# duckdb/duckdb-vss

Measured on AMD Instinct MI355X. Metric: queries/sec at recall@10, 10M×768 FLOAT top-10; index build rows/sec, higher is better.
Workload: dtype f32

## Files before the change

duckdb-vss_amd/__init__.py:

```python
import ctypes as C
import os
import subprocess

import numpy as np

HERE = os.path.dirname(os.path.abspath(__file__))
ROOT = os.path.dirname(HERE)
LIB_PATH = os.environ.get("VSS_LIBRARY") or os.path.join(HERE, "libvssgpu.so")
CSRC = os.path.join(HERE, "csrc")

METRICS = {"l2sq": 0, "cosine": 1, "ip": 2}
FUNCTIONS = {"array_distance": 0, "array_cosine_distance": 1, "array_negative_inner_product": 2}
FREE_KEY = np.iinfo(np.int64).max

HIPCC_FLAGS = ["--offload-arch=gfx950", "-O3", "-std=c++17", "-ffp-contract=off", "-fPIC", "-Wno-int-to-pointer-cast"]


TRANSLATION_UNITS = ["vss_engine.hip", "vss_exchange.hip", "kernels_l2sq.hip", "kernels_cosine.hip", "kernels_ip.hip",
                     "kernels_boxes_l2sq.hip", "kernels_boxes_cosine.hip", "kernels_boxes_ip.hip",
                     "kernels_setboxes_l2sq.hip", "kernels_setboxes_cosine.hip", "kernels_setboxes_ip.hip"]


def build_library(force=False, extra_flags=(), out=None):
    out = out or os.path.join(HERE, "libvssgpu.so")
# ... 80 lines not shown
    "vss_set_label_column64": (_int, [_vp, _u32, _u64, _vp, _u64]),
    "vss_set_label_column64_device": (_int, [_vp, _u32, _u64, _vp, _u64]),
    "vss_label_column_width": (_u32, [_vp, _u32]),
    "vss_search_batch_by_label_box64": (_int, [_vp, _vp, _u64, _u64, _u64, _vp, _u64, _vp, _vp, _int, _u64, _vp, _vp, _vp, _vp]),
    "vss_search_batch_by_label_box64_device": (_int, [_vp, _vp, _u64, _u64, _u64, _vp, _u64, _vp, _vp, _int, _u64, _vp, _vp, _vp,
                                                      _vp]),
    "vss_search_batch_by_label_set_box": (_int, [_vp, _vp, _u64, _u64, _u64, _u32, _vp, _u32, _vp, _u64, _vp, _vp, _int, _u64, _vp, _vp,
                                                 _vp, _vp]),
    "vss_search_batch_by_label_set_box_device": (_int, [_vp, _vp, _u64, _u64, _u64, _u32, _vp, _u32, _vp, _u64, _vp, _vp, _int, _u64,
                                                        _vp, _vp, _vp, _vp]),
    "vss_last_exact_fallbacks": (_u64, [_vp]),
    "vss_last_search_stats": (_int, [_vp, _vp]),
    "vss_last_search_shape": (_int, [_vp, _vp]),
    "vss_last_search_prescore": (_int, [_vp, _vp]),
    "vss_last_search_prescore_descent": (_int, [_vp, _vp]),
    "vss_last_search_query_stats": (_int, [_vp, _vp, _u64]),
    "vss_timing": (_int, [_vp, _vp, _int]),
    "vss_build_work": (_int, [_vp, _vp]),
    "vss_remove_batch": (_int, [_vp, _vp, _u64, _vp]),
    "vss_compact": (_int, [_vp]),
    "vss_compact_ex": (_int, [_vp, _int, _vp]),
    "vss_size": (_u64, [_vp]),
    "vss_nodes": (_u64, [_vp]),
    "vss_build_progress": (_int, [_vp, _vp, _vp]),
    "vss_capacity": (_u64, [_vp]),
    "vss_max_level": (_u64, [_vp]),
    "vss_memory_usage": (_u64, [_vp]),
    "vss_dimensions": (_u64, [_vp]),
    "vss_metric": (_int, [_vp]),
    "vss_level_stats": (_int, [_vp, _u64, _vp]),
# ... 538 lines not shown

    def last_exact_fallbacks(self):
        return int(self.lib.vss_last_exact_fallbacks(self.h))

    def timing(self, reset=False):
        out = np.zeros(6, dtype=np.float64)
        self._check(self.lib.vss_timing(self.h, _p(out), int(reset)))
        return dict(search_kernel_ms=out[0], build_phase_a_ms=out[1], build_phase_b_ms=out[2], build_wall_ms=out[3],
                    build_batches=int(out[4]), build_retries=int(out[5]))

    def build_work(self):
        out = np.zeros(3, dtype=np.uint64)
        self._check(self.lib.vss_build_work(self.h, _p(out)))
        return dict(insert_distances=int(out[0]), insert_expansions=int(out[1]), link_distances=int(out[2]))

    def last_query_stats(self, nq):
        out = np.zeros((nq, 2), dtype=np.uint32)
        self._check(self.lib.vss_last_search_query_stats(self.h, _p(out), nq))
        return out

    def remove(self, rowids):
        rowids = np.ascontiguousarray(rowids, dtype=np.int64)
        n = _u64(0)
        self._check(self.lib.vss_remove_batch(self.h, _p(rowids), len(rowids), C.byref(n)))
        return n.value

    def compact(self, reorder=True):
        done = C.c_int(0)
        self._check(self.lib.vss_compact_ex(self.h, 1 if reorder else 0, C.byref(done)))
        return bool(done.value)
# ... 79 lines not shown
```

duckdb-vss_amd/csrc/hnsw_kernels.h:

```cpp
#pragma once
#include "wave_primitives.h"
#include "engine_layout.h"
#include "prescore_bound.h"
#include "filter_groups.h"
#include "label_filter.h"
#include <type_traits>

namespace vss {

constexpr int64_t FREE_KEY = 0x7FFFFFFFFFFFFFFFll;

constexpr uint64_t FILTER_PER_QUERY = 1ull << 63;
constexpr uint64_t FILTER_BY_LABEL = 1ull << 62;
constexpr uint64_t FILTER_BY_RANGE = 1ull << 61;
constexpr uint64_t FILTER_BY_SET = 1ull << 60;
constexpr uint64_t FILTER_FLAGS = FILTER_PER_QUERY | FILTER_BY_LABEL | FILTER_BY_RANGE | FILTER_BY_SET;
constexpr uint64_t FILTER_BY_BOX = FILTER_BY_RANGE | FILTER_BY_SET;
__host__ __device__ constexpr bool filter_by_box(uint64_t filter_bits) {
	return (filter_bits & FILTER_BY_BOX) == FILTER_BY_BOX;
}
constexpr uint64_t FILTER_BY_BOX64 = FILTER_BY_LABEL | FILTER_BY_RANGE | FILTER_BY_SET;
__host__ __device__ constexpr bool filter_by_box64(uint64_t filter_bits) {
	return (filter_bits & FILTER_BY_BOX64) == FILTER_BY_BOX64;
}
// ... 349 lines not shown
		return fresh;
	}
	__device__ __forceinline__ void clear_fresh() {
		fresh = 0;
	}
};

template <int MT, int NCH, int R, bool LATE = false>
struct SoloScorer {
	static constexpr bool touches_rows = LATE, touches_lists = LATE, helpers_touch = false;
	static constexpr bool bounds_descent = false;
	__device__ __forceinline__ void at_level(int) const {
	}
	__device__ __forceinline__ void at_bound(float) const {
	}
	__device__ __forceinline__ bool latency_mode() const {
		return false;
	}
	template <typename F>
	__device__ __forceinline__ void operator()(const WaveLds &lds, const RowSpace &sp, float qa2, int n, F before_loads
	                                           VSS_WC_ARG) const {
		if constexpr (LATE) {
			if (n <= 0)
				before_loads();
			wave_distances<MT, NCH, R>(sp, lds.q, qa2, lds.ids, n, lds.dist, before_loads);
		} else {
			before_loads();
			wave_distances<MT, NCH, R>(sp, lds.q, qa2, lds.ids, n, lds.dist);
		}
	}
// ... 4 lines not shown
	const int per = ((n + T - 1) / T + RG - 1) & ~(RG - 1);
	lo = wave * per < n ? wave * per : n;
	hi = lo + per < n ? lo + per : n;
}
struct NoListCache {};
template <int MT, int NCH, int R, int T>
struct TeamScorer {
	static constexpr bool touches_rows = false, touches_lists = true, helpers_touch = true;
	__device__ __forceinline__ bool latency_mode() const {
		return false;
	}
	static constexpr bool bounds_descent = false;
	__device__ __forceinline__ void at_level(int) const {
	}
	__device__ __forceinline__ void at_bound(float) const {
	}
	TeamBox *box;
	template <typename F, class Cache>
	__device__ __forceinline__ void run(const WaveLds &lds, const RowSpace &sp, float qa2, int n, F before_loads, Cache &cache,
	                                    bool touch) const {
		if (n <= 0) {
			before_loads();
			return;
		}
		if (lane_id() == 0)
			box->n = n, box->qa2 = qa2;
		__syncthreads();
		int lo, hi;
		team_share(sp, n, T, 0, lo, hi);
		wave_distances<MT, NCH, R>(sp, lds.q, qa2, lds.ids, hi, lds.dist, before_loads);
// ... 192 lines not shown
#pragma unroll
		for (int r = 0; r < RR; ++r)
			accumulate4<MT>(q, x[ch][r], ab[r], b2[r]);
	}
	transposed_reduce64<RR>(ab);
	if (MT == 1)
		transposed_reduce64<RR>(b2);
	constexpr int PER = 64 / RR;
	int j = pos[0];
#pragma unroll
	for (int r = 1; r < RR; ++r)
		j = (int)(lane / PER) == r ? pos[r] : j;
	if ((lane % PER) == 0)
		out[j] = finish_distance<MT>(ab[0], qa2, b2[0]);
}


typedef __attribute__((address_space(3))) unsigned long long lds_u64;
typedef __attribute__((address_space(3))) uint32_t lds_u32;
typedef __attribute__((address_space(3))) float lds_f32;
typedef uint32_t lds_u32x4 __attribute__((ext_vector_type(4)));
typedef __attribute__((address_space(3))) lds_u32x4 lds_u32x4_as3;
#define VSS_LDS_PTR(type, ptr) ((type *)(uint32_t)(uintptr_t)(ptr))
#define VSS_LDS_LOAD(type, ptr) __hip_atomic_load(VSS_LDS_PTR(type, ptr), __ATOMIC_RELAXED, __HIP_MEMORY_SCOPE_WORKGROUP)
#define VSS_LDS_STORE(type, ptr, v) __hip_atomic_store(VSS_LDS_PTR(type, ptr), (v), __ATOMIC_RELAXED, __HIP_MEMORY_SCOPE_WORKGROUP)
#define VSS_LDS_ADD(type, ptr, v) __hip_atomic_fetch_add(VSS_LDS_PTR(type, ptr), (v), __ATOMIC_RELAXED, __HIP_MEMORY_SCOPE_WORKGROUP)
#ifdef VSS_RELAXED_MAILBOX
#define VSS_MB_RELEASE __ATOMIC_RELAXED
#define VSS_MB_ACQUIRE __ATOMIC_RELAXED
#else
// ... 108 lines not shown
	uint32_t no_requests;
	uint32_t touch_ok;
	uint32_t prescore_ok;
	unsigned long long *descent_counters;
	mutable uint32_t crew_on = 0;
	mutable uint32_t level = 0;
	mutable float hop_bound = __builtin_inff();
	mutable uint32_t hop_filtered = 0;
	static constexpr bool bounds_descent = PRE;
	__device__ __forceinline__ void at_level(int l) const {
		level = (uint32_t)l;
	}
	__device__ __forceinline__ void at_bound(float bound) const {
		hop_bound = (PRE && descent_counters) ? bound : __builtin_inff();
	}
	__device__ __forceinline__ void add_descent_counts(uint32_t rows, uint32_t rejected) const {
		if (PRE && descent_counters && rows && lane_id() == 0) {
			atomicAdd(descent_counters, (unsigned long long)rows);
			atomicAdd(descent_counters + 1, (unsigned long long)rejected);
		}
	}

	__device__ __forceinline__ bool wants_requests() const {
		return !(crew_on && no_requests);
	}

	__device__ __forceinline__ bool latency_mode() const {
		return crew_on != 0 && touch_ok != 0;
	}
	__device__ __forceinline__ uint32_t active_walkers() const {
// ... 320 lines not shown
		VSS_TICK(tk1);
		VSS_ACC(t_pick, tk0, tk1);
		uint32_t first_cells;
		const bool have_first = can_prefetch && ahead.find(cs, first_cells);
		VSS_COUNT(t_look, have_first ? 1u : 0u);
		const int n = gather_neighbors<true>(gv, lds, cs, level, have_first, first_cells);
		VSS_TICK(tk2);
		VSS_ACC(t_gather, tk1, tk2);
		if (n < 0)
			return LEVEL_VISITED_OVERFLOW;
		auto look_ahead = request_ahead;
		if (n == 0) {
			look_ahead();
			continue;
		}
		if constexpr (TOUCH_H)
			score.run(lds, gv.sp, qa2, n, look_ahead, ahead, (lds.touch_lines & 0xFFu) && can_prefetch);
		else
			score(lds, gv.sp, qa2, n, look_ahead VSS_WC_PASS);
		wc.distances += n;
		VSS_TICK(tk3);
		VSS_ACC(t_dist, tk2, tk3);
		if constexpr (TOUCH) {
			if ((lds.touch_lines & 0xFFu) && can_prefetch) {
				touch.retire();
				VSS_COUNT(t_slice, (unsigned)__builtin_popcount(ahead.fresh_bits()));
				touch.issue(ahead, gv.sp, lds.touch_lines & 0xFFu);
			}
		}
		bool touch_lists = false;
// ... 317 lines not shown
				pool.end(nb, gv.sp, n_next);
			return LEVEL_INTERNAL;
		}
		if (next == EMPTY_SLOT)
			break;
		L.mark_expanded(pos);
		request_ahead();
		VSS_TICK(ta1);
		VSS_ACC(t_accept, ta0, ta1);
		b = nb;
		n_cur = n_next;
	}
	return LEVEL_OK;
}

template <int MT, int NCH, int R>
__device__ __forceinline__ int refine_candidates(const GraphView &gv, WaveLds &lds, int count, int needed,
                                                 WorkCounters &wc) {
	const int lane = lane_id();
	if (count < needed) {
		for (int i = lane; i < count; i += 64) {
			lds.kept_s[i] = lds.cand_s[i];
			lds.kept_d[i] = lds.cand_d[i];
		}
		wave_sync();
		return count;
	}
	if (lane == 0) {
		lds.kept_s[0] = lds.cand_s[0];
		lds.kept_d[0] = lds.cand_d[0];
	}
	wave_sync();
	int submitted = 1, consumed = 1;
	while (submitted < needed && consumed < count) {
		const uint32_t cs = lds.cand_s[consumed];
		const float cd = lds.cand_d[consumed];
		stage_row(lds.q2, gv.sp.vectors + (size_t)cs * gv.sp.V, gv.sp.V);
		const float c2 = MT == 1 ? wave_query_norm(gv.sp, lds.q2) : 0.f;
		const int pass = R * (64 >> gv.sp.logG);
		bool bad = false;
		for (int off = 0; off < submitted && !bad; off += pass) {
			const int n = submitted - off < pass ? submitted - off : pass;
			wave_distances<MT, NCH, R>(gv.sp, lds.q2, c2, lds.kept_s + off, n, lds.dist);
			wc.distances += n;
			for (int o = 0; o < n; o += 64) {
				const bool b = (o + lane < n) && (lds.dist[o + lane] < cd);
				bad = bad || (__ballot(b) != 0ull);
			}
			wave_sync();
		}
		if (!bad) {
			if (lane == 0) {
				lds.kept_s[submitted] = cs;
				lds.kept_d[submitted] = cd;
			}
			submitted++;
// ... 672 lines not shown
	uint32_t *counters;
	uint32_t req_capacity;
	uint32_t *global_hash;
	const uint32_t *work;
	uint32_t *node_status;
	uint32_t node_req_cap;
	unsigned long long *work_stats;
	const uint32_t *row_slot;
	const uint32_t *row_src;
	const float4 *pending;
	uint32_t *parked;
	uint32_t parked_stride;
	float *list_buf;
	uint32_t list_cap;
	uint32_t cand_lds_cap;
};

#ifndef VSS_BUILD_WAVES_PER_EU
#define VSS_BUILD_WAVES_PER_EU(NCH, E) ((NCH) == 6 ? 2 : (((E) >= 8 || (NCH) == 4) ? 3 : 4))
#endif
template <int MT, int NCH, int R, int E>
__global__ __launch_bounds__(64) __attribute__((amdgpu_waves_per_eu(VSS_BUILD_WAVES_PER_EU(NCH, E), 8))) void
k_build_phase_a(BuildArgs a) {
	extern __shared__ __attribute__((aligned(16))) unsigned char smem[];
	const int lane = lane_id();
	const uint32_t node = a.work ? a.work[blockIdx.x] : blockIdx.x;
	const uint32_t slot = a.row_slot ? a.row_slot[node] : a.first_slot + node;
	const uint32_t src = a.row_src ? a.row_src[node] : EMPTY_SLOT;
	WaveLds lds;
	carve_lds(lds, smem, a.hash_log2, a.gv.sp.V, a.list_cap_max, a.cand_lds_cap, a.global_hash);
	uint32_t *req_l = reinterpret_cast<uint32_t *>(
	    smem + wave_lds_bytes(a.hash_log2, a.gv.sp.V, a.list_cap_max, a.cand_lds_cap, a.global_hash == nullptr));
	float *req_dd = reinterpret_cast<float *>(req_l + a.node_req_cap);
	stage_row(lds.q, src == EMPTY_SLOT ? a.gv.sp.vectors + (size_t)slot * a.gv.sp.V : a.pending + (size_t)src * a.gv.sp.V,
	          a.gv.sp.V);
	const float qa2 = MT == 1 ? wave_query_norm(a.gv.sp, lds.q) : 0.f;
	WorkCounters wc = {};
	const int target = a.levels[slot];
	const SoloScorer<MT, NCH, R> score;
	uint32_t closest = descend<MT>(a.gv, lds, qa2, a.entry, a.max_level, target, score, wc);
	typename std::conditional<E == 0, MemList, WaveList<(E == 0 ? 1 : E)>>::type L;
	if constexpr (E == 0)
		L.bind(a.list_buf + (size_t)blockIdx.x * 2 * a.list_cap,
		       reinterpret_cast<uint32_t *>(a.list_buf + (size_t)blockIdx.x * 2 * a.list_cap) + a.list_cap);
	CandQueue unused_queue;
	uint32_t n_req = 0;
	for (int level = target < a.max_level ? target : a.max_level; level >= 0; --level) {
		if (level_search_impl<MT, true, false, 1>(a.gv, lds, qa2, closest, slot, level, a.top_limit, L, unused_queue, score, wc) !=
		    LEVEL_OK) {
			if (lane == 0) {
				a.node_status[node] = 1;
				atomicExch(&a.counters[3], 1u);
			}
			return;
		}
		if constexpr (E == 0) {
			for (int i = lane; i < L.size; i += 64)
				L.s[i] &= ~EXPANDED_BIT;
			lds.cand_d = L.d;
			lds.cand_s = L.s;
		} else {
			L.dump(lds.cand_d, lds.cand_s);
		}
		wave_sync();
		const int kept = refine_candidates<MT, NCH, R>(a.gv, lds, L.size, a.gv.M, wc);
		uint32_t *mine = src == EMPTY_SLOT ? a.gv.list_ptr(slot, level)
		                                   : a.parked + (size_t)node * a.parked_stride + (size_t)level * a.list_cap_max;
		const uint32_t cap = a.gv.list_cap(level);
		for (uint32_t i = lane; i < cap; i += 64)
			mine[i] = i < (uint32_t)kept ? lds.kept_s[i] : EMPTY_SLOT;
		for (int i = lane; i < kept; i += 64) {
			const uint32_t t = lds.kept_s[i];
			req_l[n_req + i] =
			    t == slot ? EMPTY_SLOT : (level == 0 ? t : a.gv.list_id_base + a.gv.upper_off[t] + (level - 1));
			req_dd[n_req + i] = lds.kept_d[i];
		}
		n_req += kept;
		closest = lds.kept_s[0];
		wave_sync();
	}
	uint32_t base = 0;
	if (lane == 0) {
		base = atomicAdd(&a.counters[0], n_req);
		a.node_status[node] = 0;
		atomicAdd(&a.work_stats[0], (unsigned long long)wc.distances);
		atomicAdd(&a.work_stats[1], (unsigned long long)wc.cycles);
	}
	base = read_lane(base, 0);
	for (uint32_t i = lane; i < n_req; i += 64) {
		const uint32_t idx = base + i;
		if (idx < a.req_capacity) {
			a.req_list[idx] = req_l[i];
			a.req_src[idx] = slot | (src == EMPTY_SLOT ? 0u : REUSED_SOURCE);
			a.req_d[idx] = req_dd[i];
		}
	}
}

struct LinkArgs {
	GraphView gv;
	uint32_t *req_list;
// ... 424 lines not shown
```

duckdb-vss_amd/csrc/row_codes.h:

```cpp
#pragma once
#include "prescore_bound.h"

#include <algorithm>

namespace vss {

VSS_PRESCORE_HD inline float row_code_scale(float amax) {
	const float scale = amax / 127.0f;
	return (scale >= 1.17549435e-38f && scale < INFINITY) ? scale : 0.f;
}
VSS_PRESCORE_HD inline int row_code_of(float x, float scale) {
	float c = rintf(x / scale);
	c = c > 127.f ? 127.f : c;
	c = c < -127.f ? -127.f : c;
	return (int)c;
}
VSS_PRESCORE_HD inline double row_code_residual(float x, float scale, int code) {
	return (double)x - (double)scale * (double)code;
}
VSS_PRESCORE_HD inline RowCodeMeta row_code_meta(float scale, double e2, double n2, bool finite) {
	RowCodeMeta m;
	m.scale = scale, m.spare = 0;
	m.norm = (float)sqrt(n2);
	if (!finite || !(scale > 0.f) || !(e2 == e2)) {
// ... 18 lines not shown
	}
	void mark(uint64_t first, uint64_t end) {
		if (first >= end)
			return;
		if (!any())
			lo = first, hi = end;
		else
			lo = std::min(lo, first), hi = std::max(hi, end);
	}
	void mark_all() {
		lo = 0, hi = ~0ull;
	}
	void clear() {
		lo = hi = 0;
	}
	bool take(uint64_t rows, uint64_t &first, uint64_t &end) {
		first = lo, end = std::min(hi, rows);
		const bool work = first < end;
		if (hi <= rows)
			clear();
		else if (work)
			lo = rows;
		return work;
	}
};

#if defined(__HIPCC__)
__global__ __launch_bounds__(256) void k_encode_rows(const float4 *vectors, uint32_t V, uint64_t first, uint64_t end, uint32_t *codes,
                                                     RowCodeMeta *meta) {
	const uint32_t lane = threadIdx.x & 63u;
	const uint64_t waves = (uint64_t)gridDim.x * (blockDim.x >> 6);
	for (uint64_t slot = first + (uint64_t)blockIdx.x * (blockDim.x >> 6) + (threadIdx.x >> 6); slot < end; slot += waves) {
		const float4 *row = vectors + slot * V;
		float amax = 0.f;
		bool finite = true;
		for (uint32_t c = lane; c < V; c += 64) {
			const float4 x = row[c];
			const float a = fmaxf(fmaxf(fabsf(x.x), fabsf(x.y)), fmaxf(fabsf(x.z), fabsf(x.w)));
			finite = finite && fabsf(x.x) < INFINITY && fabsf(x.y) < INFINITY && fabsf(x.z) < INFINITY && fabsf(x.w) < INFINITY;
			amax = fmaxf(amax, a);
		}
		for (int off = 32; off; off >>= 1)
			amax = fmaxf(amax, __shfl_xor(amax, off));
		finite = __all(finite);
		const float scale = finite ? row_code_scale(amax) : 0.f;
		double e2 = 0.0, n2 = 0.0;
		for (uint32_t c = lane; c < V; c += 64) {
			const float4 x = row[c];
			const float xs[4] = {x.x, x.y, x.z, x.w};
			uint32_t word = 0;
#pragma unroll
			for (int k = 0; k < 4; ++k) {
				const int code = scale > 0.f ? row_code_of(xs[k], scale) : 0;
				const double r = scale > 0.f ? row_code_residual(xs[k], scale, code) : 0.0;
				e2 += r * r;
				n2 += (double)xs[k] * (double)xs[k];
				word |= ((uint32_t)code & 0xFFu) << (8 * k);
			}
			codes[slot * V + c] = word;
		}
		for (int off = 32; off; off >>= 1) {
			e2 += __shfl_xor(e2, off);
			n2 += __shfl_xor(n2, off);
		}
		if (lane == 0)
			meta[slot] = row_code_meta(scale, e2, n2, finite);
	}
}
#endif

}
```

duckdb-vss_amd/csrc/vss_engine.hip:

```cpp
#include <hip/hip_runtime.h>

#include <algorithm>
#include <atomic>
#include <chrono>
#include <cmath>
#include <cstdarg>
#include <cstdio>
#include <cstdlib>
#include <cstring>
#include <condition_variable>
#include <mutex>
#include <shared_mutex>
#include <string>
#include <thread>
#include <vector>

#define VSS_ENGINE_TU
#include "../../include/vssgpu.h"
#include "launchers.h"
#include "host_logic.h"
#include "filter_groups.h"
#include "label_filter.h"
#include "exact_filtered_kernels.h"
#include "filter_route_kernels.h"
// ... 617 lines not shown
		if (codes_stale.take(count, first, end)) {
			const uint32_t grid = (uint32_t)std::min<uint64_t>((end - first + 3) / 4, (uint64_t)n_cus * 16);
			hipLaunchKernelGGL(k_encode_rows, dim3(grid), dim3(256), 0, s, reinterpret_cast<const float4 *>(d_vectors.p), V, first, end,
			                   d_codes.p, d_code_meta.p);
			hipError_t status = hipGetLastError();
			if (status == hipSuccess)
				status = hipStreamSynchronize(s);
			if (status != hipSuccess) {
				codes_stale = before;
				throw HipError {status, "k_encode_rows"};
			}
		}
		return true;
	}

	void refresh_codes() noexcept {
		try {
			(void)ensure_codes(stream, true);
		} catch (...) {
			(void)hipGetLastError();
		}
	}

	uint64_t last_stats[4] = {0, 0, 0, 0};
	uint32_t last_shape[8] = {0, 0, 0, 0, 0, 0, 0, 0};
	std::vector<uint32_t> last_query_stats;
	double timing[6] = {0, 0, 0, 0, 0, 0};
	hipEvent_t ev[4] = {nullptr, nullptr, nullptr, nullptr};
	void ensure_events() {
		for (auto &e : ev)
// ... 49 lines not shown
		gv.keys = d_keys.p;
		gv.list_id_base = (uint32_t)capacity;
		gv.filter = nullptr;
		gv.filter_bits = 0;
		gv.twins = lists_may_repeat ? 1u : 0u;
		return gv;
	}

	void release() {
		d_vectors.free(), d_links0.free(), d_links_up.free(), d_upper_off.free(), d_list_owner.free();
		d_levels.free(), d_keys.free();
		clear_labels();
		free_codes();
		d_req_list.free(), d_req_src.free(), d_req_rank.free(), d_sorted_src.free(), d_touched.free();
		d_list_count.free(), d_list_offset.free(), d_counters.free(), d_req_d.free(), d_sorted_d.free();
		d_node_status.free(), d_work_build.free(), d_work_stats.free(), d_build_list.free();
		if (h_debug)
			(void)hipHostFree(h_debug);
		h_debug = nullptr;
		d_pending.free(), d_row_slot.free(), d_row_src.free(), d_parked.free();
		d_global_hash.free(), d_row_norm2.free(), d_q_norm2.free(), d_scores.free(), d_best_s.free(), d_qpad.free();
		d_best_i.free(), d_cand_s.free(), d_cand_cnt.free(), d_cand_i.free();
		d_norm_ext.free(), d_certified.free(), d_redo_map.free();
		d_xf_lists.free(), d_xf_counts.free(), d_xf_tables.free();
		exact_filter_bytes.store(0, std::memory_order_relaxed);
		if (h_counters)
			(void)hipHostFree(h_counters);
		h_counters = nullptr;
		for (auto &e : ev) {
			if (e)
				(void)hipEventDestroy(e);
// ... 394 lines not shown
				solo_row = i;
		std::vector<uint64_t> sizes = batch_schedule(first, max_level, lv, n, max_batch, growth_div, solo_row);
		uint64_t biggest = 0, top_lv = 0;
		for (uint64_t b : sizes)
			biggest = std::max(biggest, b);
		for (uint64_t i = 0; i != n; ++i)
			top_lv = std::max<uint64_t>(top_lv, lv[i]);
		ensure_build_scratch(biggest, top_lv);
		uint64_t appended = 0;
		progress_linked.store(0, std::memory_order_relaxed);
		progress_total.store(n, std::memory_order_relaxed);
		uint64_t done = 0;
		int rc = VSS_OK;
		ensure_events();
		bool pending_b = false;
		auto wall0 = std::chrono::steady_clock::now();
		for (uint64_t b : sizes) {
			const uint64_t slot0 = slot_of(done);
			if (slot0 == 0 && first == 0 && done == 0) {
				entry = 0;
				max_level = levels_h[0];
				done += b;
				count = first + (appended += b);
				progress_linked.store(done, std::memory_order_relaxed);
				continue;
			}
			uint32_t bump = 0;
			uint32_t level_hi = 0, batch_reused = 0;
			for (uint64_t j = 0; j != b; ++j) {
				level_hi = std::max<uint32_t>(level_hi, lv[done + j]);
				batch_reused += reuse && st_src[done + j] != EMPTY_SLOT;
			}
			BuildArgs reuse_args;
			if (batch_reused) {
				reuse_args.gv = view();
				reuse_args.levels = d_levels.p;
				reuse_args.max_level = max_level;
				reuse_args.list_cap_max = list_cap_max();
				reuse_args.row_slot = d_row_slot.p + done, reuse_args.row_src = d_row_src.p + done;
				reuse_args.parked_stride = (level_hi + 1) * list_cap_max();
				d_parked.ensure((uint64_t)b * reuse_args.parked_stride, 0, stream);
				reuse_args.parked = d_parked.p;
				hipLaunchKernelGGL(k_reuse_lists, dim3((uint32_t)b), dim3(64), 0, stream, reuse_args, 0);
			}
			HIP_TRY(hipMemsetAsync(d_counters.p, 0, 8 * sizeof(uint32_t), stream));
			d_node_status.ensure(b, 0, stream);
			if (h_node_status.size() < b)
				h_node_status.resize(b);
			std::vector<uint32_t> work;
			for (;;) {
				BuildArgs a;
				a.gv = view();
				a.first_slot = (uint32_t)slot0;
				a.n_nodes = (uint32_t)b;
				a.levels = d_levels.p;
				a.entry = entry;
				a.max_level = max_level;
				a.top_limit = top_limit();
				a.hash_log2 = hash_log2_for(top_limit(), bump);
				a.list_cap_max = list_cap_max();
// ... 7 lines not shown
				a.node_req_cap = (uint32_t)(M * (level_hi + 1));
				a.work_stats = d_work_stats.p;
				a.row_slot = reuse ? d_row_slot.p + done : nullptr;
				a.row_src = reuse ? d_row_src.p + done : nullptr;
				a.pending = reinterpret_cast<const float4 *>(d_pending.p);
				a.parked = batch_reused ? d_parked.p : nullptr;
				a.parked_stride = (level_hi + 1) * list_cap_max();
				const bool list_in_hbm = top_limit() > 64 * MAX_LIST_REGS;
				a.cand_lds_cap = list_in_hbm ? 16 : a.top_limit;
				a.list_cap = list_in_hbm ? a.top_limit : 0;
				a.list_buf = nullptr;
				if (list_in_hbm) {
					d_build_list.ensure((uint64_t)grid * 2 * a.list_cap, 0, stream);
					a.list_buf = d_build_list.p;
				}
				const uint32_t lds = wave_lds_bytes(a.hash_log2, V, a.list_cap_max, a.cand_lds_cap, !a.global_hash) +
				                     align16(a.node_req_cap * 4) * 2;
				HIP_TRY(hipEventRecord(ev[0], stream));
				launch_by_metric<BuildArgs>(launch_phase_a<0>, launch_phase_a<1>, launch_phase_a<2>, a,
				                            launch_cfg(grid, lds, top_limit()));
				HIP_TRY(hipEventRecord(ev[1], stream));
				HIP_TRY(hipMemcpyAsync(h_counters, d_counters.p, 8 * sizeof(uint32_t), hipMemcpyDeviceToHost, stream));
				HIP_TRY(hipStreamSynchronize(stream));
				{
					float ms = 0;
					HIP_TRY(hipEventElapsedTime(&ms, ev[0], ev[1]));
					timing[1] += ms;
					if (pending_b) {
						HIP_TRY(hipEventElapsedTime(&ms, ev[2], ev[3]));
						timing[2] += ms;
// ... 47 lines not shown
				hipLaunchKernelGGL(k_link_alloc, dim3(gb), dim3(tb), 0, stream, l);
				hipLaunchKernelGGL(k_link_scatter, dim3(gb), dim3(tb), 0, stream, l);
				const uint32_t lds = wave_lds_bytes(l.hash_log2, V, l.list_cap_max, l.list_cap_max + 1);
				launch_by_metric<LinkArgs>(launch_phase_b<0>, launch_phase_b<1>, launch_phase_b<2>, l,
				                           launch_cfg(std::min<uint32_t>(n_req, 65536), lds, 64));
				HIP_TRY(hipEventRecord(ev[3], stream));
				pending_b = true;
			}
			for (uint64_t j = 0; batch_reused && j != b; ++j) {
				const uint32_t src = st_src[done + j], slot = st_slot[done + j];
				if (src == EMPTY_SLOT)
					continue;
				const uint64_t stride = (uint64_t)V * 4;
				HIP_TRY(hipMemcpyAsync(d_vectors.p + slot * stride, d_pending.p + src * stride, stride * 4,
				                       hipMemcpyDeviceToDevice, stream));
				codes_stale.mark(slot, (uint64_t)slot + 1);
				HIP_TRY(hipMemcpyAsync(d_keys.p + slot, &pending_keys[src], 8, hipMemcpyHostToDevice, stream));
			}
			for (uint64_t j = 0; j != b; ++j) {
				if ((int)lv[done + j] > max_level) {
					max_level = lv[done + j];
					entry = (uint32_t)slot_of(done + j);
				}
			}
			for (uint64_t j = 0; j != b; ++j)
				appended += !reuse || st_src[done + j] == EMPTY_SLOT;
			tombstones -= batch_reused;
			done += b;
			count = first + appended;
			progress_linked.store(done, std::memory_order_relaxed);
		}
		HIP_TRY(hipStreamSynchronize(stream));
// ... 1920 lines not shown
     "a launch is issued when its predecessor on the device starts to drain"},
    {"search.list_lds", 0, 2, [](vss_index *h, int64_t v) { h->search_list_lds = (uint32_t)v; },
     "candidate lists of limits 513-4096 in LDS: 0 never (HBM), 1 when the workgroup keeps its walkers, 2 whenever one walker fits"},
    {"search.prescore", 0, 2,
     [](vss_index *h, int64_t v) {
	     h->search_prescore = (uint32_t)v;
	     if (!h->search_prescore)
		     h->free_codes();
	     else if (h->stream)
		     h->refresh_codes();
     },
     "scoring waves reject rows on exact bounds from 8-bit row codes before reading their f32 components: 0 never, 1 at limits of "
     "at most 256, 2 in every pipelined launch"},
    {"search.prescore_descent", 0, 1, [](vss_index *h, int64_t v) { h->search_prescore_descent = v != 0; },
     "in launches that filter on row codes, the greedy descent's rows are bounded against its closest distance too"},
};
const char *set_option_checked(vss_index *h, const char *name, int64_t value) {
	for (const OptionRule &r : OPTION_RULES) {
		if (std::strcmp(r.name, name))
			continue;
		if (value < r.lo || value > r.hi)
			return "value out of range";
		if (!std::strcmp(name, "search.visited_cells_per_limit") && value != 0 && value < 4)
			return "value out of range";
		const uint32_t waves = !std::strcmp(name, "search.waves") ? (uint32_t)value : h->search_waves;
		const uint32_t walkers = !std::strcmp(name, "search.walkers") ? (uint32_t)value : h->search_walkers;
		if (walkers && walkers >= waves)
			return "at least one scoring wave must remain";
		r.apply(h, value);
		return nullptr;
// ... 42 lines not shown
		return VSS_ERROR;
	}
	std::memset(h->h_debug, 0, 128 * sizeof(uint32_t));
#endif
	hipDeviceProp_t prop;
	if (hipGetDeviceProperties(&prop, device) == hipSuccess && prop.multiProcessorCount > 0)
		h->n_cus = (uint32_t)prop.multiProcessorCount;
	static const struct { const char *env, *option; } ENV_OPTIONS[] = {
	    {"VSS_SEARCH_WAVES", "search.waves"}, {"VSS_SEARCH_WALKERS", "search.walkers"}, {"VSS_SEARCH_SPEC", "search.lookahead"},
	    {"VSS_SEARCH_SOLO", "search.solo"}, {"VSS_SEARCH_SOLO_MAX", "search.solo_max_queries"}, {"VSS_SEARCH_TEAM", "search.team"},
	    {"VSS_SEARCH_CREW", "search.crew"}, {"VSS_SEARCH_PIPELINED", "search.pipelined"},
	    {"VSS_SEARCH_WIDE_LISTS", "search.wide_lists"}, {"VSS_VISITED_COMPACT", "search.visited_compact"},
	    {"VSS_SEARCH_RETRY_IN_PLACE", "search.retry_in_place"}, {"VSS_HASH_LDS_MAX_LOG2", "search.visited_lds_log2_max"},
	    {"VSS_VISITED_PER_LIMIT", "search.visited_cells_per_limit"}, {"VSS_PROBE_FLAG_WAIT", "search.probe_flag_wait"},
	    {"VSS_SEARCH_LIST_LDS", "search.list_lds"}, {"VSS_SEARCH_PRESCORE", "search.prescore"},
	    {"VSS_SEARCH_PRESCORE_DESCENT", "search.prescore_descent"},
	};
	for (const auto &e : ENV_OPTIONS)
		if (const char *t = getenv(e.env)) {
			if (const char *why = set_option_checked(h, e.option, (int64_t)atoll(t)))
				fprintf(stderr, "vssgpu: %s=%s ignored (%s: %s)\n", e.env, t, e.option, why);
		}
	if (const char *t = getenv("VSS_SEARCH_REG_QUEUE"))
		h->search_reg_queue = atoi(t) != 0;
	if (const char *t = getenv("VSS_SEARCH_REG_QUEUE_MAX"))
		h->reg_queue_max_limit = (uint32_t)std::max(0, std::min(64 * MAX_LIST_REGS, atoi(t)));
	if (const char *t = getenv("VSS_FORCE_LOOPING"))
		h->force_looping = atoi(t) != 0;
	if (const char *t = getenv("VSS_EXACT_PROBE"))
		h->exact_probe = (uint32_t)atoi(t);
	if (const char *t = getenv("VSS_EXACT_KERNEL"))
// ... 996 lines not shown
int vss_build_work(vss_index *h, uint64_t *out3) {
	VSS_SHARED(h, {
		std::memset(out3, 0, 3 * sizeof(uint64_t));
		if (h->d_work_stats.p) {
			HIP_TRY(hipStreamSynchronize(h->stream));
			unsigned long long v[4];
			HIP_TRY(hipMemcpy(v, h->d_work_stats.p, sizeof v, hipMemcpyDeviceToHost));
			out3[0] = v[0];
			out3[1] = v[1];
			out3[2] = v[2];
		}
		return VSS_OK;
	})
}

int vss_timing(vss_index *h, double *out6, int reset) {
	VSS_SHARED(h, {
		std::lock_guard<std::mutex> lk(h->stats_mu);
		std::memcpy(out6, h->timing, sizeof h->timing);
		if (reset)
			std::memset(h->timing, 0, sizeof h->timing);
		return VSS_OK;
	})
}

int vss_last_search_query_stats(vss_index *h, uint32_t *out, uint64_t nq) {
	VSS_SHARED(h, {
		std::lock_guard<std::mutex> lk(h->stats_mu);
		if (h->last_query_stats.size() < nq * 2)
			return h->fail("no per-query stats recorded for %llu queries", (unsigned long long)nq);
// ... 222 lines not shown
```

include/vssgpu.h:

```cpp
#ifndef VSSGPU_H
#define VSSGPU_H
#include <stdint.h>
#ifdef __cplusplus
extern "C" {
#endif

typedef struct vss_index vss_index;

enum { VSS_OK = 0, VSS_ERROR = 1 };

enum { VSS_METRIC_L2SQ = 0, VSS_METRIC_COSINE = 1, VSS_METRIC_IP = 2 };

enum { VSS_FN_ARRAY_DISTANCE = 0, VSS_FN_ARRAY_COSINE_DISTANCE = 1, VSS_FN_ARRAY_NEGATIVE_INNER_PRODUCT = 2 };

#define VSS_FREE_KEY INT64_MAX


int vss_create(uint64_t dim, int metric, uint64_t M, uint64_t M0, uint64_t ef_construction, uint64_t ef_search,
               int device, vss_index **out);
void vss_destroy(vss_index *index);
const char *vss_last_error(vss_index *index);
int vss_set_stream(vss_index *index, void *hip_stream);
int vss_synchronize(vss_index *index);

// ... 128 lines not shown
                                           const uint64_t *n_groups, uint64_t n_bits, const uint32_t *const *d_group_of,
                                           int64_t *const *d_out_rowids, float *const *d_out_distances,
                                           uint32_t *const *d_out_counts);
int vss_search_batch_end(vss_index *index, int context);
int vss_search_exact_batch(vss_index *index, const float *queries, uint64_t n_queries, uint64_t k,
                           int64_t *out_rowids, float *out_distances, uint32_t *out_counts);
int vss_search_exact_batch_device(vss_index *index, const float *d_queries, uint64_t n_queries, uint64_t k,
                                  int64_t *d_out_rowids, float *d_out_distances, uint32_t *d_out_counts);
uint64_t vss_last_exact_fallbacks(vss_index *index);
int vss_last_search_stats(vss_index *index, uint64_t *out4);
int vss_last_search_shape(vss_index *index, uint32_t *out8);
int vss_last_search_prescore(vss_index *index, uint64_t *out4);
int vss_last_search_prescore_descent(vss_index *index, uint64_t *out2);
int vss_timing(vss_index *index, double *out6, int reset);
int vss_build_work(vss_index *index, uint64_t *out3);
int vss_last_search_query_stats(vss_index *index, uint32_t *out, uint64_t n_queries);


int vss_remove_batch(vss_index *index, const int64_t *rowids, uint64_t count, uint64_t *out_removed);
int vss_compact(vss_index *index);
int vss_compact_ex(vss_index *index, int reorder, int *out_reordered);

uint64_t vss_size(vss_index *index);
uint64_t vss_nodes(vss_index *index);
uint64_t vss_capacity(vss_index *index);
uint64_t vss_max_level(vss_index *index);
uint64_t vss_memory_usage(vss_index *index);
uint64_t vss_dimensions(vss_index *index);
int vss_metric(vss_index *index);
int vss_level_stats(vss_index *index, uint64_t level, uint64_t *out4);
// ... 44 lines not shown
```

Measured before the change: 1.728 million.

## Prescore candidate rows with 8-bit codes during bulk HNSW build inserts

Adds a BuildScorer that, once the insert search's candidate list is full, bounds each neighbor row using the 8-bit row codes against the current radius. Full f32 distances are computed only for survivors. The build now keeps the codes current by encoding newly linked rows and reused slots each batch, and can optionally prescore inside refine_candidates (mode 2). This aims to cut f32 vector reads during index construction, at the cost of extra encode kernels, more register pressure, and new counters and atomics.

Result: no change. 1.730 million (median of 4 runs) (+0.2%).

```diff
diff --git a/duckdb-vss_amd/__init__.py b/duckdb-vss_amd/__init__.py
--- a/duckdb-vss_amd/__init__.py
+++ b/duckdb-vss_amd/__init__.py
@@ -118,6 +118,7 @@
     "vss_last_search_shape": (_int, [_vp, _vp]),
     "vss_last_search_prescore": (_int, [_vp, _vp]),
     "vss_last_search_prescore_descent": (_int, [_vp, _vp]),
+    "vss_build_prescore": (_int, [_vp, _vp]),
     "vss_last_search_query_stats": (_int, [_vp, _vp, _u64]),
     "vss_timing": (_int, [_vp, _vp, _int]),
     "vss_build_work": (_int, [_vp, _vp]),
@@ -686,6 +687,12 @@
         self._check(self.lib.vss_build_work(self.h, _p(out)))
         return dict(insert_distances=int(out[0]), insert_expansions=int(out[1]), link_distances=int(out[2]))
 
+    def build_prescore(self):
+        out = np.zeros(5, dtype=np.uint64)
+        self._check(self.lib.vss_build_prescore(self.h, _p(out)))
+        return dict(search_prescored=int(out[0]), search_rejected=int(out[1]), refine_prescored=int(out[2]),
+                    refine_rejected=int(out[3]), refine_distances=int(out[4]))
+
     def last_query_stats(self, nq):
         out = np.zeros((nq, 2), dtype=np.uint32)
         self._check(self.lib.vss_last_search_query_stats(self.h, _p(out), nq))
diff --git a/duckdb-vss_amd/csrc/hnsw_kernels.h b/duckdb-vss_amd/csrc/hnsw_kernels.h
--- a/duckdb-vss_amd/csrc/hnsw_kernels.h
+++ b/duckdb-vss_amd/csrc/hnsw_kernels.h
@@ -387,6 +387,8 @@
 	}
 	__device__ __forceinline__ void at_bound(float) const {
 	}
+	__device__ __forceinline__ void at_radius(float) const {
+	}
 	__device__ __forceinline__ bool latency_mode() const {
 		return false;
 	}
@@ -421,6 +423,8 @@
 	__device__ __forceinline__ void at_level(int) const {
 	}
 	__device__ __forceinline__ void at_bound(float) const {
+	}
+	__device__ __forceinline__ void at_radius(float) const {
 	}
 	TeamBox *box;
 	template <typename F, class Cache>
@@ -643,6 +647,60 @@
 	if ((lane % PER) == 0)
 		out[j] = finish_distance<MT>(ab[0], qa2, b2[0]);
 }
+template <int MT, int NCH, int R, int CR>
+__device__ __forceinline__ void wave_distances_survivors(const RowSpace &sp, const float4 *q_lds, float qa2, const uint32_t *ids,
+                                                         unsigned long long left, float *out) {
+	constexpr int SHIFT = CR == 16 ? 2 : CR == 8 ? 3 : 4;
+	static_assert(CR == 16 || CR == 8 || CR == 4, "rows of codes per claim");
+	while (left) {
+		const int have = __popcll(left);
+		if (have >= 3 && R >= 4)
+			wave_distances_picked<MT, NCH, (R >= 4 ? 4 : 1)>(sp, q_lds, qa2, ids, left, SHIFT, out);
+		else if (have >= 2)
+			wave_distances_picked<MT, NCH, 2>(sp, q_lds, qa2, ids, left, SHIFT, out);
+		else
+			wave_distances_picked<MT, NCH, 1>(sp, q_lds, qa2, ids, left, SHIFT, out);
+	}
+}
+
+template <int MT, int NCH, int R, int CR, int RS = R>
+struct BuildScorer {
+	static constexpr bool touches_rows = false, touches_lists = false, helpers_touch = false;
+	static constexpr bool bounds_descent = false;
+	PrescoreView pv;
+	uint32_t dim;
+	mutable float bound = __builtin_inff();
+	mutable uint32_t pre = 0, rejected = 0;
+	__device__ __forceinline__ void at_level(int) const {
+	}
+	__device__ __forceinline__ void at_bound(float) const {
+	}
+	__device__ __forceinline__ void at_radius(float b) const {
+		bound = pv.codes ? b : __builtin_inff();
+	}
+	__device__ __forceinline__ bool latency_mode() const {
+		return false;
+	}
+	template <typename F>
+	__device__ __forceinline__ void operator()(const WaveLds &lds, const RowSpace &sp, float qa2, int n, F before_loads
+	                                           VSS_WC_ARG) const {
+		before_loads();
+		const float b = bound;
+		bound = __builtin_inff();
+		if (b < __builtin_inff()) {
+			for (int c = 0; c < n; c += CR) {
+				const int cnt = n - c < CR ? n - c : CR;
+				const unsigned long long left =
+				    prescore_codes<MT, NCH, CR>(sp, pv, dim, lds.q, qa2, lds.ids + c, cnt, b, lds.dist + c, rejected);
+				pre += (uint32_t)cnt;
+				wave_distances_survivors<MT, NCH, RS, CR>(sp, lds.q, qa2, lds.ids + c, left, lds.dist + c);
+			}
+			wave_sync();
+			return;
+		}
+		wave_distances<MT, NCH, R>(sp, lds.q, qa2, lds.ids, n, lds.dist);
+	}
+};
 
 
 typedef __attribute__((address_space(3))) unsigned long long lds_u64;
@@ -781,6 +839,8 @@
 	__device__ __forceinline__ void at_bound(float bound) const {
 		hop_bound = (PRE && descent_counters) ? bound : __builtin_inff();
 	}
+	__device__ __forceinline__ void at_radius(float) const {
+	}
 	__device__ __forceinline__ void add_descent_counts(uint32_t rows, uint32_t rejected) const {
 		if (PRE && descent_counters && rows && lane_id() == 0) {
 			atomicAdd(descent_counters, (unsigned long long)rows);
@@ -1131,6 +1191,8 @@
 			look_ahead();
 			continue;
 		}
+		if constexpr (!TOMB)
+			score.at_radius(L.size >= limit ? radius : __builtin_inff());
 		if constexpr (TOUCH_H)
 			score.run(lds, gv.sp, qa2, n, look_ahead, ahead, (lds.touch_lines & 0xFFu) && can_prefetch);
 		else
@@ -1478,9 +1540,14 @@
 	return LEVEL_OK;
 }
 
-template <int MT, int NCH, int R>
+struct RefinePrescore {
+	PrescoreView pv;
+	uint32_t dim;
+	uint32_t pre = 0, rejected = 0;
+};
+template <int MT, int NCH, int R, bool PRE = false, int CR = 16, int RS = R>
 __device__ __forceinline__ int refine_candidates(const GraphView &gv, WaveLds &lds, int count, int needed,
-                                                 WorkCounters &wc) {
+                                                 WorkCounters &wc, RefinePrescore *rp = nullptr) {
 	const int lane = lane_id();
 	if (count < needed) {
 		for (int i = lane; i < count; i += 64) {
@@ -1500,10 +1567,36 @@
 		const uint32_t cs = lds.cand_s[consumed];
 		const float cd = lds.cand_d[consumed];
 		stage_row(lds.q2, gv.sp.vectors + (size_t)cs * gv.sp.V, gv.sp.V);
-		const float c2 = MT == 1 ? wave_query_norm(gv.sp, lds.q2) : 0.f;
+		bool filter = false;
+		if constexpr (PRE)
+			filter = rp->pv.codes != nullptr && cd < __builtin_inff();
+		const float c2 = (MT == 1 || (MT == 2 && filter)) ? wave_query_norm(gv.sp, lds.q2) : 0.f;
 		const int pass = R * (64 >> gv.sp.logG);
 		bool bad = false;
-		for (int off = 0; off < submitted && !bad; off += pass) {
+		if constexpr (PRE) {
+			if (filter) {
+				constexpr int PER = 64 / CR;
+				constexpr unsigned long long PASS_BITS = PER * R >= 64 ? ~0ull : (1ull << (PER * R % 64)) - 1ull;
+				static_assert(NCH >= 2 && PER * R <= 64 && CR % R == 0, "full-wave rows; a block of codes is a whole number of f32 passes");
+				for (int blk = 0; blk < submitted && !bad; blk += CR) {
+					const int bn = submitted - blk < CR ? submitted - blk : CR;
+					const unsigned long long left =
+					    prescore_codes<MT, NCH, CR>(gv.sp, rp->pv, rp->dim, lds.q2, c2, lds.kept_s + blk, bn, cd, lds.dist, rp->rejected);
+					rp->pre += (uint32_t)bn;
+					for (int off = 0; off < bn && !bad; off += R) {
+						const int n = bn - off < R ? bn - off : R;
+						const unsigned long long part = (left >> (PER * off)) & PASS_BITS;
+						wave_distances_survivors<MT, NCH, RS, CR>(gv.sp, lds.q2, c2, lds.kept_s + blk + off, part, lds.dist + off);
+						wave_sync();
+						wc.distances += n;
+						const bool b = (lane < n) && (lds.dist[off + lane] < cd);
+						bad = __ballot(b) != 0ull;
+						wave_sync();
+					}
+				}
+			}
+		}
+		for (int off = 0; !filter && off < submitted && !bad; off += pass) {
 			const int n = submitted - off < pass ? submitted - off : pass;
 			wave_distances<MT, NCH, R>(gv.sp, lds.q2, c2, lds.kept_s + off, n, lds.dist);
 			wc.distances += n;
@@ -2206,10 +2299,21 @@
 	float *list_buf;
 	uint32_t list_cap;
 	uint32_t cand_lds_cap;
+	PrescoreView prescore = {nullptr, nullptr, nullptr};
+	uint32_t prescore_refine = 0;
 };
 
 #ifndef VSS_BUILD_WAVES_PER_EU
 #define VSS_BUILD_WAVES_PER_EU(NCH, E) ((NCH) == 6 ? 2 : (((E) >= 8 || (NCH) == 4) ? 3 : 4))
+#endif
+#ifndef VSS_BUILD_CODE_ROWS
+#define VSS_BUILD_CODE_ROWS(NCH, E) (((NCH) == 3 && (E) == 4) ? 4 : (((NCH) <= 3 && (E) <= 4) || ((NCH) == 4 && (E) >= 8)) ? 8 : 16)
+#endif
+#ifndef VSS_BUILD_REFINE_PRESCORE
+#define VSS_BUILD_REFINE_PRESCORE(MT, NCH, E) (!((MT) == 1 && (NCH) == 3 && (E) == 4))
+#endif
+#ifndef VSS_BUILD_SURVIVOR_ROWS
+#define VSS_BUILD_SURVIVOR_ROWS(NCH, E) ((((NCH) == 3 && (E) <= 4) || ((NCH) == 4 && (E) >= 8)) ? 2 : 4)
 #endif
 template <int MT, int NCH, int R, int E>
 __global__ __launch_bounds__(64) __attribute__((amdgpu_waves_per_eu(VSS_BUILD_WAVES_PER_EU(NCH, E), 8))) void
@@ -2226,10 +2330,22 @@
 	float *req_dd = reinterpret_cast<float *>(req_l + a.node_req_cap);
 	stage_row(lds.q, src == EMPTY_SLOT ? a.gv.sp.vectors + (size_t)slot * a.gv.sp.V : a.pending + (size_t)src * a.gv.sp.V,
 	          a.gv.sp.V);
-	const float qa2 = MT == 1 ? wave_query_norm(a.gv.sp, lds.q) : 0.f;
 	WorkCounters wc = {};
 	const int target = a.levels[slot];
-	const SoloScorer<MT, NCH, R> score;
+	constexpr bool PRE = E >= 1 && (NCH == 2 || NCH == 3 || NCH == 4 || NCH == 6);
+	constexpr int CR = VSS_BUILD_CODE_ROWS(NCH, E), RS = VSS_BUILD_SURVIVOR_ROWS(NCH, E) < R ? VSS_BUILD_SURVIVOR_ROWS(NCH, E) : R;
+	typename std::conditional<PRE, BuildScorer<MT, (PRE ? NCH : 2), R, CR, RS>, SoloScorer<MT, NCH, R>>::type score;
+	constexpr bool PRE_REFINE = PRE && VSS_BUILD_REFINE_PRESCORE(MT, NCH, E);
+	RefinePrescore refine_pre;
+	if constexpr (PRE)
+		score.pv = a.prescore, score.dim = a.gv.dim;
+	if constexpr (PRE_REFINE) {
+		refine_pre.pv = a.prescore, refine_pre.dim = a.gv.dim;
+		if (!a.prescore_refine)
+			refine_pre.pv.codes = nullptr;
+	}
+	const float qa2 = (MT == 1 || (PRE && MT == 2 && a.prescore.codes)) ? wave_query_norm(a.gv.sp, lds.q) : 0.f;
+	uint32_t refine_distances = 0;
 	uint32_t closest = descend<MT>(a.gv, lds, qa2, a.entry, a.max_level, target, score, wc);
 	typename std::conditional<E == 0, MemList, WaveList<(E == 0 ? 1 : E)>>::type L;
 	if constexpr (E == 0)
@@ -2255,7 +2371,9 @@
 			L.dump(lds.cand_d, lds.cand_s);
 		}
 		wave_sync();
-		const int kept = refine_candidates<MT, NCH, R>(a.gv, lds, L.size, a.gv.M, wc);
+		const uint32_t before_refine = wc.distances;
+		const int kept = refine_candidates<MT, NCH, R, PRE_REFINE, CR, RS>(a.gv, lds, L.size, a.gv.M, wc, &refine_pre);
+		refine_distances += wc.distances - before_refine;
 		uint32_t *mine = src == EMPTY_SLOT ? a.gv.list_ptr(slot, level)
 		                                   : a.parked + (size_t)node * a.parked_stride + (size_t)level * a.list_cap_max;
 		const uint32_t cap = a.gv.list_cap(level);
@@ -2277,6 +2395,18 @@
 		a.node_status[node] = 0;
 		atomicAdd(&a.work_stats[0], (unsigned long long)wc.distances);
 		atomicAdd(&a.work_stats[1], (unsigned long long)wc.cycles);
+		if (a.prescore.counters)
+			atomicAdd(&a.prescore.counters[4], (unsigned long long)refine_distances);
+		if constexpr (PRE) {
+			if (a.prescore.codes) {
+				atomicAdd(&a.prescore.counters[0], (unsigned long long)score.pre);
+				atomicAdd(&a.prescore.counters[1], (unsigned long long)score.rejected);
+				if (PRE_REFINE && a.prescore_refine) {
+					atomicAdd(&a.prescore.counters[2], (unsigned long long)refine_pre.pre);
+					atomicAdd(&a.prescore.counters[3], (unsigned long long)refine_pre.rejected);
+				}
+			}
+		}
 	}
 	base = read_lane(base, 0);
 	for (uint32_t i = lane; i < n_req; i += 64) {
diff --git a/duckdb-vss_amd/csrc/row_codes.h b/duckdb-vss_amd/csrc/row_codes.h
--- a/duckdb-vss_amd/csrc/row_codes.h
+++ b/duckdb-vss_amd/csrc/row_codes.h
@@ -56,6 +56,16 @@
 	void clear() {
 		lo = hi = 0;
 	}
+	void encoded(uint64_t first, uint64_t end) {
+		if (!any() || first >= end)
+			return;
+		if (first <= lo && end > lo)
+			lo = std::min(end, hi);
+		if (end >= hi && first < hi)
+			hi = std::max(first, lo);
+		if (!any())
+			clear();
+	}
 	bool take(uint64_t rows, uint64_t &first, uint64_t &end) {
 		first = lo, end = std::min(hi, rows);
 		const bool work = first < end;
@@ -68,46 +78,57 @@
 };
 
 #if defined(__HIPCC__)
+__device__ __forceinline__ void encode_row(const float4 *vectors, uint32_t V, uint64_t slot, uint32_t *codes, RowCodeMeta *meta,
+                                           uint32_t lane) {
+	const float4 *row = vectors + slot * V;
+	float amax = 0.f;
+	bool finite = true;
+	for (uint32_t c = lane; c < V; c += 64) {
+		const float4 x = row[c];
+		const float a = fmaxf(fmaxf(fabsf(x.x), fabsf(x.y)), fmaxf(fabsf(x.z), fabsf(x.w)));
+		finite = finite && fabsf(x.x) < INFINITY && fabsf(x.y) < INFINITY && fabsf(x.z) < INFINITY && fabsf(x.w) < INFINITY;
+		amax = fmaxf(amax, a);
+	}
+	for (int off = 32; off; off >>= 1)
+		amax = fmaxf(amax, __shfl_xor(amax, off));
+	finite = __all(finite);
+	const float scale = finite ? row_code_scale(amax) : 0.f;
+	double e2 = 0.0, n2 = 0.0;
+	for (uint32_t c = lane; c < V; c += 64) {
+		const float4 x = row[c];
+		const float xs[4] = {x.x, x.y, x.z, x.w};
+		uint32_t word = 0;
+#pragma unroll
+		for (int k = 0; k < 4; ++k) {
+			const int code = scale > 0.f ? row_code_of(xs[k], scale) : 0;
+			const double r = scale > 0.f ? row_code_residual(xs[k], scale, code) : 0.0;
+			e2 += r * r;
+			n2 += (double)xs[k] * (double)xs[k];
+			word |= ((uint32_t)code & 0xFFu) << (8 * k);
+		}
+		codes[slot * V + c] = word;
+	}
+	for (int off = 32; off; off >>= 1) {
+		e2 += __shfl_xor(e2, off);
+		n2 += __shfl_xor(n2, off);
+	}
+	if (lane == 0)
+		meta[slot] = row_code_meta(scale, e2, n2, finite);
+}
 __global__ __launch_bounds__(256) void k_encode_rows(const float4 *vectors, uint32_t V, uint64_t first, uint64_t end, uint32_t *codes,
                                                      RowCodeMeta *meta) {
 	const uint32_t lane = threadIdx.x & 63u;
 	const uint64_t waves = (uint64_t)gridDim.x * (blockDim.x >> 6);
-	for (uint64_t slot = first + (uint64_t)blockIdx.x * (blockDim.x >> 6) + (threadIdx.x >> 6); slot < end; slot += waves) {
-		const float4 *row = vectors + slot * V;
-		float amax = 0.f;
-		bool finite = true;
-		for (uint32_t c = lane; c < V; c += 64) {
-			const float4 x = row[c];
-			const float a = fmaxf(fmaxf(fabsf(x.x), fabsf(x.y)), fmaxf(fabsf(x.z), fabsf(x.w)));
-			finite = finite && fabsf(x.x) < INFINITY && fabsf(x.y) < INFINITY && fabsf(x.z) < INFINITY && fabsf(x.w) < INFINITY;
-			amax = fmaxf(amax, a);
-		}
-		for (int off = 32; off; off >>= 1)
-			amax = fmaxf(amax, __shfl_xor(amax, off));
-		finite = __all(finite);
-		const float scale = finite ? row_code_scale(amax) : 0.f;
-		double e2 = 0.0, n2 = 0.0;
-		for (uint32_t c = lane; c < V; c += 64) {
-			const float4 x = row[c];
-			const float xs[4] = {x.x, x.y, x.z, x.w};
-			uint32_t word = 0;
-#pragma unroll
-			for (int k = 0; k < 4; ++k) {
-				const int code = scale > 0.f ? row_code_of(xs[k], scale) : 0;
-				const double r = scale > 0.f ? row_code_residual(xs[k], scale, code) : 0.0;
-				e2 += r * r;
-				n2 += (double)xs[k] * (double)xs[k];
-				word |= ((uint32_t)code & 0xFFu) << (8 * k);
-			}
-			codes[slot * V + c] = word;
-		}
-		for (int off = 32; off; off >>= 1) {
-			e2 += __shfl_xor(e2, off);
-			n2 += __shfl_xor(n2, off);
-		}
-		if (lane == 0)
-			meta[slot] = row_code_meta(scale, e2, n2, finite);
-	}
+	for (uint64_t slot = first + (uint64_t)blockIdx.x * (blockDim.x >> 6) + (threadIdx.x >> 6); slot < end; slot += waves)
+		encode_row(vectors, V, slot, codes, meta, lane);
+}
+__global__ __launch_bounds__(256) void k_encode_slots(const float4 *vectors, uint32_t V, const uint32_t *slots, const uint32_t *src,
+                                                      uint32_t skip, uint64_t n, uint64_t rows, uint32_t *codes, RowCodeMeta *meta) {
+	const uint32_t lane = threadIdx.x & 63u;
+	const uint64_t waves = (uint64_t)gridDim.x * (blockDim.x >> 6);
+	for (uint64_t i = (uint64_t)blockIdx.x * (blockDim.x >> 6) + (threadIdx.x >> 6); i < n; i += waves)
+		if (src[i] != skip && slots[i] < rows)
+			encode_row(vectors, V, slots[i], codes, meta, lane);
 }
 #endif
 
diff --git a/duckdb-vss_amd/csrc/vss_engine.hip b/duckdb-vss_amd/csrc/vss_engine.hip
--- a/duckdb-vss_amd/csrc/vss_engine.hip
+++ b/duckdb-vss_amd/csrc/vss_engine.hip
@@ -655,6 +655,36 @@
 		return true;
 	}
 
+	uint32_t build_prescore = 1;
+	DevBuf<unsigned long long> d_build_prescore;
+	bool build_codes_begin() noexcept {
+		if (!build_prescore || top_limit() > 64 * MAX_LIST_REGS)
+			return false;
+		try {
+			return ensure_codes(stream, true);
+		} catch (...) {
+			(void)hipGetLastError();
+			return false;
+		}
+	}
+	bool encode_linked_range(uint64_t first, uint64_t end) noexcept {
+		if (first >= end)
+			return true;
+		const uint32_t grid = (uint32_t)std::min<uint64_t>((end - first + 3) / 4, (uint64_t)n_cus * 16);
+		hipLaunchKernelGGL(k_encode_rows, dim3(grid), dim3(256), 0, stream, reinterpret_cast<const float4 *>(d_vectors.p), V, first, end,
+		                   d_codes.p, d_code_meta.p);
+		if (hipGetLastError() != hipSuccess)
+			return false;
+		codes_stale.encoded(first, end);
+		return true;
+	}
+	bool encode_batch_reused(const uint32_t *d_slots, const uint32_t *d_src, uint64_t n) noexcept {
+		const uint32_t grid = (uint32_t)std::min<uint64_t>((n + 3) / 4, (uint64_t)n_cus * 16);
+		hipLaunchKernelGGL(k_encode_slots, dim3(grid), dim3(256), 0, stream, reinterpret_cast<const float4 *>(d_vectors.p), V, d_slots,
+		                   d_src, EMPTY_SLOT, n, (uint64_t)capacity, d_codes.p, d_code_meta.p);
+		return hipGetLastError() == hipSuccess;
+	}
+
 	void refresh_codes() noexcept {
 		try {
 			(void)ensure_codes(stream, true);
@@ -734,7 +764,7 @@
 		free_codes();
 		d_req_list.free(), d_req_src.free(), d_req_rank.free(), d_sorted_src.free(), d_touched.free();
 		d_list_count.free(), d_list_offset.free(), d_counters.free(), d_req_d.free(), d_sorted_d.free();
-		d_node_status.free(), d_work_build.free(), d_work_stats.free(), d_build_list.free();
+		d_node_status.free(), d_work_build.free(), d_work_stats.free(), d_build_list.free(), d_build_prescore.free();
 		if (h_debug)
 			(void)hipHostFree(h_debug);
 		h_debug = nullptr;
@@ -1159,6 +1189,9 @@
 		int rc = VSS_OK;
 		ensure_events();
 		bool pending_b = false;
+		d_build_prescore.ensure(8, 0, stream, 0);
+		bool codes_live = build_codes_begin();
+		uint64_t coded = count;
 		auto wall0 = std::chrono::steady_clock::now();
 		for (uint64_t b : sizes) {
 			const uint64_t slot0 = slot_of(done);
@@ -1189,6 +1222,10 @@
 				hipLaunchKernelGGL(k_reuse_lists, dim3((uint32_t)b), dim3(64), 0, stream, reuse_args, 0);
 			}
 			HIP_TRY(hipMemsetAsync(d_counters.p, 0, 8 * sizeof(uint32_t), stream));
+			if (codes_live && coded < count) {
+				codes_live = encode_linked_range(coded, count);
+				coded = count;
+			}
 			d_node_status.ensure(b, 0, stream);
 			if (h_node_status.size() < b)
 				h_node_status.resize(b);
@@ -1226,6 +1263,8 @@
 					d_build_list.ensure((uint64_t)grid * 2 * a.list_cap, 0, stream);
 					a.list_buf = d_build_list.p;
 				}
+				a.prescore = PrescoreView {codes_live ? d_codes.p : nullptr, codes_live ? d_code_meta.p : nullptr, d_build_prescore.p};
+				a.prescore_refine = build_prescore == 2 ? 1u : 0u;
 				const uint32_t lds = wave_lds_bytes(a.hash_log2, V, a.list_cap_max, a.cand_lds_cap, !a.global_hash) +
 				                     align16(a.node_req_cap * 4) * 2;
 				HIP_TRY(hipEventRecord(ev[0], stream));
@@ -1303,8 +1342,15 @@
 				const uint64_t stride = (uint64_t)V * 4;
 				HIP_TRY(hipMemcpyAsync(d_vectors.p + slot * stride, d_pending.p + src * stride, stride * 4,
 				                       hipMemcpyDeviceToDevice, stream));
-				codes_stale.mark(slot, (uint64_t)slot + 1);
+				if (!codes_live)
+					codes_stale.mark(slot, (uint64_t)slot + 1);
 				HIP_TRY(hipMemcpyAsync(d_keys.p + slot, &pending_keys[src], 8, hipMemcpyHostToDevice, stream));
+			}
+			if (codes_live && batch_reused && !encode_batch_reused(d_row_slot.p + done, d_row_src.p + done, b)) {
+				codes_live = false;
+				for (uint64_t j = 0; j != b; ++j)
+					if (st_src[done + j] != EMPTY_SLOT)
+						codes_stale.mark(st_slot[done + j], (uint64_t)st_slot[done + j] + 1);
 			}
 			for (uint64_t j = 0; j != b; ++j) {
 				if ((int)lv[done + j] > max_level) {
@@ -3255,6 +3301,9 @@
      "at most 256, 2 in every pipelined launch"},
     {"search.prescore_descent", 0, 1, [](vss_index *h, int64_t v) { h->search_prescore_descent = v != 0; },
      "in launches that filter on row codes, the greedy descent's rows are bounded against its closest distance too"},
+    {"build.prescore", 0, 2, [](vss_index *h, int64_t v) { h->build_prescore = (uint32_t)v; },
+     "the bulk build rejects rows on the same bounds before reading their f32 components: 0 never, 1 in the insert searches, 2 in "
+     "refine_ as well (needs search.prescore != 0: the codes are shared)"},
 };
 const char *set_option_checked(vss_index *h, const char *name, int64_t value) {
 	for (const OptionRule &r : OPTION_RULES) {
@@ -3327,7 +3376,7 @@
 	    {"VSS_SEARCH_RETRY_IN_PLACE", "search.retry_in_place"}, {"VSS_HASH_LDS_MAX_LOG2", "search.visited_lds_log2_max"},
 	    {"VSS_VISITED_PER_LIMIT", "search.visited_cells_per_limit"}, {"VSS_PROBE_FLAG_WAIT", "search.probe_flag_wait"},
 	    {"VSS_SEARCH_LIST_LDS", "search.list_lds"}, {"VSS_SEARCH_PRESCORE", "search.prescore"},
-	    {"VSS_SEARCH_PRESCORE_DESCENT", "search.prescore_descent"},
+	    {"VSS_SEARCH_PRESCORE_DESCENT", "search.prescore_descent"}, {"VSS_BUILD_PRESCORE", "build.prescore"},
 	};
 	for (const auto &e : ENV_OPTIONS)
 		if (const char *t = getenv(e.env)) {
@@ -4354,6 +4403,20 @@
 	})
 }
 
+int vss_build_prescore(vss_index *h, uint64_t *out5) {
+	VSS_SHARED(h, {
+		std::memset(out5, 0, 5 * sizeof(uint64_t));
+		if (h->d_build_prescore.p) {
+			HIP_TRY(hipStreamSynchronize(h->stream));
+			unsigned long long v[5];
+			HIP_TRY(hipMemcpy(v, h->d_build_prescore.p, sizeof v, hipMemcpyDeviceToHost));
+			for (int i = 0; i != 5; ++i)
+				out5[i] = v[i];
+		}
+		return VSS_OK;
+	})
+}
+
 int vss_timing(vss_index *h, double *out6, int reset) {
 	VSS_SHARED(h, {
 		std::lock_guard<std::mutex> lk(h->stats_mu);
diff --git a/include/vssgpu.h b/include/vssgpu.h
--- a/include/vssgpu.h
+++ b/include/vssgpu.h
@@ -166,6 +166,7 @@
 int vss_last_search_prescore_descent(vss_index *index, uint64_t *out2);
 int vss_timing(vss_index *index, double *out6, int reset);
 int vss_build_work(vss_index *index, uint64_t *out3);
+int vss_build_prescore(vss_index *index, uint64_t *out5);
 int vss_last_search_query_stats(vss_index *index, uint32_t *out, uint64_t n_queries);
 
 
```
